# limix/CellRegMap

Hardware: AMD Instinct MI355X
Metric: variant-tests/sec (interaction test) (higher is better)
Workload: dtype f64

## Files before the change

cellregmap_amd/csrc/api_core.hip:

```cpp
#include <dlfcn.h>

#include <algorithm>
#include <atomic>
#include <cstdarg>
#include <mutex>

#include <map>

#include "crm_internal.h"
#include "eigh.h"

namespace crm {

static thread_local std::string g_error;

void set_error(const char* fmt, ...) {
    char buf[1024];
    va_list ap;
    va_start(ap, fmt);
    vsnprintf(buf, sizeof buf, fmt, ap);
    va_end(ap);
    g_error = buf;
}

const char* last_error_text() { return g_error.c_str(); }

namespace {
struct Roctx {
    int (*push)(const char*) = nullptr;
    int (*pop)() = nullptr;
    Roctx() {
        void* h = dlopen("librocprofiler-sdk-roctx.so", RTLD_LAZY | RTLD_GLOBAL);
        if (!h) h = dlopen("librocprofiler-sdk-roctx.so.1", RTLD_LAZY | RTLD_GLOBAL);
        if (!h) return;
        push = reinterpret_cast<int (*)(const char*)>(dlsym(h, "roctxRangePushA"));
        pop = reinterpret_cast<int (*)()>(dlsym(h, "roctxRangePop"));
        if (!push || !pop) push = nullptr, pop = nullptr;
    }
};
const Roctx& roctx() {
    static Roctx r;
    return r;
}
bool ranges_on() {
    static const bool on = getenv("CRM_ROCTX") || getenv("ROCP_TOOL_LIBRARIES") || getenv("ROCPROFILER_LIBRARY_CTOR");
    return on;
}
}

void trace_push(const char* name) {
    if (ranges_on() && roctx().push) roctx().push(name);
}
void trace_pop() {
    if (ranges_on() && roctx().pop) roctx().pop();
}

static bool poison_mode() {
    static const bool on = getenv("CRM_POISON") && atoi(getenv("CRM_POISON")) != 0;
    return on;
}
static constexpr size_t REDZONE = 4096;
static std::atomic<long> g_overruns{0};
long overruns_detected() { return g_overruns.load(); }
static std::atomic<long> g_live_bytes{0};
long live_device_bytes() { return g_live_bytes.load(); }

static void check_redzone(const void* ptr, size_t bytes) {
    if (!ptr || !poison_mode()) return;
    std::vector<unsigned char> rz(REDZONE);
    if (hipMemcpy(rz.data(), static_cast<const char*>(ptr) + bytes, REDZONE, hipMemcpyDeviceToHost) != hipSuccess) return;
    for (size_t i = 0; i < REDZONE; i++) {
        if (rz[i] != 0xFF) {
            g_overruns++;
            fprintf(stderr, "[crm] CRM_POISON: write past the end of a %zu-byte device buffer (first touched byte at +%zu)\n",
                    bytes, i);
            break;
        }
    }
}

static hipStream_t fill_stream() {
    static std::mutex mu;
    static std::map<int, hipStream_t> streams;
    int dev = 0;
    if (hipGetDevice(&dev) != hipSuccess) return nullptr;
    std::lock_guard<std::mutex> lock(mu);
    auto it = streams.find(dev);
    if (it != streams.end()) return it->second;
    hipStream_t st = nullptr;
    if (hipStreamCreateWithFlags(&st, hipStreamNonBlocking) != hipSuccess) st = nullptr;
    streams[dev] = st;
    return st;
}

int DevBuf::ensure(size_t need) {
    if (need <= bytes) return CRM_OK;
    if (ptr) {
        check_redzone(ptr, bytes);
        CRM_HIP(hipFree(ptr));
        g_live_bytes -= (long)bytes;
        ptr = nullptr;
        bytes = 0;
    }
    const size_t total = need + REDZONE;
    hipError_t e = hipMalloc(&ptr, total);
    if (e == hipErrorOutOfMemory && trim_idle_workspaces() > 0) {
        (void)hipGetLastError();
        e = hipMalloc(&ptr, total);
    }
    if (e != hipSuccess) {
        ptr = nullptr;
        (void)hipGetLastError();
        set_error("device allocation of %zu bytes failed: %s", need, hipGetErrorString(e));
        return CRM_ERR_HIP;
    }
    bytes = need;
    static std::atomic<unsigned long> allocations{0};
    serial = ++allocations;
    g_live_bytes += (long)need;
    hipStream_t fs = fill_stream();
    CRM_HIP(hipMemsetAsync(ptr, poison_mode() ? 0xFF : 0, total, fs));
    CRM_HIP(hipStreamSynchronize(fs));
    return CRM_OK;
}

static std::mutex g_ctx_mutex;
static std::vector<crm_ctx*> g_contexts;

static size_t trim_context(crm_ctx* c) {
    if (!c->eigh_ws || c->eigh_ws_busy) return 0;
    size_t freed = 0;
    for (const DevBuf* b : {&c->eigh_ws->A, &c->eigh_ws->Vt, &c->eigh_ws->Vc, &c->eigh_ws->QA, &c->eigh_ws->QB}) freed += b->bytes;
    *c->eigh_ws = EighWork();
    return freed;
}

EighWork* acquire_eigh_workspace(crm_ctx* c) {
    std::lock_guard<std::mutex> lock(g_ctx_mutex);
    if (!c->eigh_ws) c->eigh_ws = new EighWork();
    c->eigh_ws_busy = true;
    return c->eigh_ws;
}

void release_eigh_workspace(crm_ctx* c) {
    std::lock_guard<std::mutex> lock(g_ctx_mutex);
    c->eigh_ws_busy = false;
}

size_t trim_idle_workspaces() {
    std::lock_guard<std::mutex> lock(g_ctx_mutex);
    size_t freed = 0;
    for (crm_ctx* c : g_contexts) freed += trim_context(c);
    return freed;
}
void DevBuf::release() {
    if (ptr) check_redzone(ptr, bytes);
    if (ptr) (void)hipFree(ptr);
    g_live_bytes -= (long)bytes;
    ptr = nullptr;
    bytes = 0;
    serial = 0;
}

int upload_padded(hipStream_t st, double* dst, long ld_dst, long rows_pad, const double* src,
                  long ld_src, long rows, long cols) {
    CRM_HIP(hipMemsetAsync(dst, 0, sizeof(double) * rows_pad * ld_dst, st));
    if (rows > 0 && cols > 0)
        CRM_HIP(hipMemcpy2DAsync(dst, ld_dst * sizeof(double), src, ld_src * sizeof(double),
                                 cols * sizeof(double), rows, hipMemcpyHostToDevice, st));
    return CRM_OK;
}

}

using namespace crm;

extern "C" {

const char* crm_last_error(void) { return last_error_text(); }
const char* crm_version(void) { return "0.6.0"; }

int crm_ctx_create(int device, crm_ctx** out) {
    return crm::guarded("crm_ctx_create", [&]() -> int {
    if (!out) return CRM_ERR_ARG;
    *out = nullptr;
    int count = 0;
    CRM_HIP(hipGetDeviceCount(&count));
    if (device < 0 || device >= count) {
        set_error("crm_ctx_create: device %d not present (%d visible)", device, count);
        return CRM_ERR_ARG;
    }
    CRM_HIP(hipSetDevice(device));
    crm_ctx* c = new crm_ctx();
    c->device = device;
    if (const char* e = getenv("CRM_KIN_ROUTE")) c->kin_route = std::max(0, std::min(2, atoi(e)));
    CRM_HIP(hipStreamCreateWithFlags(&c->stream, hipStreamNonBlocking));
    CRM_HIP(hipStreamCreateWithFlags(&c->upload_stream, hipStreamNonBlocking));
    CRM_HIP(hipEventCreate(&c->ev0));
    CRM_HIP(hipEventCreate(&c->ev1));
    int prio_least = 0, prio_greatest = 0;
    CRM_HIP(hipDeviceGetStreamPriorityRange(&prio_least, &prio_greatest));
    CRM_HIP(hipStreamCreateWithPriority(&c->side_stream, hipStreamNonBlocking, prio_least));
    for (hipEvent_t* e : {&c->ev_fork, &c->ev_side, &c->ev_main, &c->ev_fits}) CRM_HIP(hipEventCreateWithFlags(e, hipEventDisableTiming));
    {
        std::lock_guard<std::mutex> lock(g_ctx_mutex);
        g_contexts.push_back(c);
    }
    *out = c;
    return CRM_OK;
    });
}

int crm_ctx_trim(crm_ctx* c) {
    return crm::guarded_on("crm_ctx_trim", c, [&]() -> int {
    if (!c) return CRM_ERR_ARG;
    CRM_HIP(hipSetDevice(c->device));
    CRM_HIP(hipStreamSynchronize(c->stream));
    if (c->side_stream) CRM_HIP(hipStreamSynchronize(c->side_stream));
    std::lock_guard<std::mutex> lock(g_ctx_mutex);
    (void)trim_context(c);
    return CRM_OK;
    });
}

void crm_ctx_destroy(crm_ctx* c) {
    try {
    if (!c) return;
    (void)hipSetDevice(c->device);
    (void)hipStreamSynchronize(c->stream);
    if (c->side_stream) (void)hipStreamSynchronize(c->side_stream);
    {
        std::lock_guard<std::mutex> lock(g_ctx_mutex);
        g_contexts.erase(std::remove(g_contexts.begin(), g_contexts.end(), c), g_contexts.end());
        delete c->eigh_ws;
        c->eigh_ws = nullptr;
    }
    c->replay_clear();
    for (auto* b : c->all_bufs()) b->release();
    for (auto& e : c->timed) {
        (void)hipEventDestroy(e.first);
        (void)hipEventDestroy(e.second);
    }
    (void)hipEventDestroy(c->ev0);
    (void)hipEventDestroy(c->ev1);
    for (hipEvent_t e : {c->ev_fork, c->ev_side, c->ev_main, c->ev_fits})
        if (e) (void)hipEventDestroy(e);
    if (c->side_stream) (void)hipStreamDestroy(c->side_stream);
    (void)hipStreamDestroy(c->stream);
    if (c->upload_stream) (void)hipStreamDestroy(c->upload_stream);
    if (c->sync_timeouts_host) (void)hipHostFree(c->sync_timeouts_host);
    delete c;
    } catch (...) {
    }
}

int crm_ctx_synchronize(crm_ctx* c) {
    return crm::guarded_on("crm_ctx_synchronize", c, [&]() -> int {
    if (!c) return CRM_ERR_ARG;
    CRM_HIP(hipSetDevice(c->device));
    CRM_HIP(hipStreamSynchronize(c->stream));
    if (c->side_stream) CRM_HIP(hipStreamSynchronize(c->side_stream));
    return CRM_OK;
    });
}

int crm_set_block_variants(crm_ctx* c, int variants) {
    return crm::guarded_on("crm_set_block_variants", c, [&]() -> int {
    if (!c || variants < 0) return CRM_ERR_ARG;
    c->block_variants = variants == 0 ? 0 : (int)round_up(variants, 128);
    return CRM_OK;
    });
}

int crm_set_null_fit_polish(crm_ctx* c, int on) {
    return crm::guarded_on("crm_set_null_fit_polish", c, [&]() -> int {
    if (!c) return CRM_ERR_ARG;
    c->polish = on != 0;
    return CRM_OK;
    });
}

int crm_set_progress_callback(crm_ctx* c, void (*callback)(long, long, void*), void* user) {
    return crm::guarded_on("crm_set_progress_callback", c, [&]() -> int {
    if (!c) return CRM_ERR_ARG;
    if (callback) c->progress[std::this_thread::get_id()] = crm_ctx::Progress{callback, user};
    else c->progress.erase(std::this_thread::get_id());
    return CRM_OK;
    });
}

int crm_set_fast_rotation(crm_ctx* c, int on) {
    return crm::guarded_on("crm_set_fast_rotation", c, [&]() -> int {
    if (!c) return CRM_ERR_ARG;
    c->fast_T = on != 0;
    return CRM_OK;
    });
}

extern "C++" {
namespace crm {
namespace {
struct FormSlot { const char* name; int value; bool set; };
FormSlot g_forms[] = {{"gram_staged", 0, false}, {"kr_no_tail", 0, false}, {"nullfit_per_wave", 0, false}, {"kin_fold", 0, false},
                      {"eigh_one_stage", 0, false}, {"nullfit_exact", 0, false}, {"donor_pairs", 0, false},
                      {"pairs_without_kinship_term", 0, false}, {"flat_kappa_milli", 0, false}, {"chase_abort", 0, false}, {"nullfit_one_per_wave", 0, false},
                      {"kin_diag", 0, false}, {"donor_pairs_rotate", 0, false}, {"rho0_positions", 0, false},
                      {"rotation_tails", 0, false}, {"woodbury_ytY", 0, false},
                      {"wb_block_order", 0, false}, {"block_fused", 0, false}, {"wb_gram_fused", 0, false},
                      {"gram_strips", 0, false}, {"side_stream", 0, false}};
std::mutex g_forms_mu;
}
int form(const char* name, int otherwise) {
    std::lock_guard<std::mutex> lock(g_forms_mu);
    for (const FormSlot& f : g_forms)
        if (strcmp(f.name, name) == 0) return f.set ? f.value : otherwise;
    return otherwise;
}
}
}

int crm_test_set_form(const char* name, int value, int reset) {
    return crm::guarded("crm_test_set_form", [&]() -> int {
    if (!name) return CRM_ERR_ARG;
    std::lock_guard<std::mutex> lock(crm::g_forms_mu);
    for (crm::FormSlot& f : crm::g_forms)
        if (strcmp(f.name, name) == 0) {
            f.value = value;
            f.set = reset == 0;
            return CRM_OK;
        }
    crm::set_error("crm_test_set_form: no kernel form is called '%s'", name);
    return CRM_ERR_ARG;
    });
}

long crm_test_tail_launches(const crm_ctx* ctx) { return ctx ? ctx->tail_launches : -1; }

long crm_test_spectrum_tail_launches(const crm_ctx* ctx) { return ctx ? ctx->spectrum_tail_launches : -1; }

long crm_test_dense_repeats(const crm_ctx* ctx) { return ctx ? ctx->dense_repeats : -1; }

long crm_test_donor_pair_blocks(const crm_ctx* ctx) { return ctx ? ctx->donor_pair_blocks : -1; }

int crm_test_gram_dma_launches(const crm_ctx* ctx, long* launches) {
    return crm::guarded("crm_test_gram_dma_launches", [&]() -> int {
    if (!ctx || !launches) return CRM_ERR_ARG;
    *launches = ctx->gram_dma_launches;
    return CRM_OK;
    });
}
int crm_test_unrelated_donor_blocks(const crm_ctx* ctx, long* blocks) {
    return crm::guarded("crm_test_unrelated_donor_blocks", [&]() -> int {
    if (!ctx || !blocks) return CRM_ERR_ARG;
    *blocks = ctx->unrelated_donor_blocks;
    return CRM_OK;
    });
}

int crm_test_fused_blocks(const crm_ctx* ctx, long* blocks) {
    return crm::guarded("crm_test_fused_blocks", [&]() -> int {
    if (!ctx || !blocks) return CRM_ERR_ARG;
    *blocks = ctx->fused_blocks;
    return CRM_OK;
    });
}

int crm_test_wb_gram_fused_blocks(const crm_ctx* ctx, long* blocks) {
    return crm::guarded("crm_test_wb_gram_fused_blocks", [&]() -> int {
    if (!ctx || !blocks) return CRM_ERR_ARG;
    *blocks = ctx->wb_gram_fused_blocks;
    return CRM_OK;
    });
}

int crm_test_side_stream_blocks(const crm_ctx* ctx, long* blocks) {
    return crm::guarded("crm_test_side_stream_blocks", [&]() -> int {
    if (!ctx || !blocks) return CRM_ERR_ARG;
    *blocks = ctx->side_stream_blocks;
    return CRM_OK;
    });
}

int crm_test_rho0_position_blocks(const crm_ctx* ctx, long* blocks) {
    return crm::guarded("crm_test_rho0_position_blocks", [&]() -> int {
    if (!ctx || !blocks) return CRM_ERR_ARG;
    *blocks = ctx->rho0_position_blocks;
    return CRM_OK;
    });
}
int crm_test_rotation_tail_launches(const crm_ctx* ctx, long* launches) {
    return crm::guarded("crm_test_rotation_tail_launches", [&]() -> int {
    if (!ctx || !launches) return CRM_ERR_ARG;
    *launches = ctx->rotation_tail_launches;
    return CRM_OK;
    });
}

long crm_test_tests_without_pair(const crm_ctx* ctx) { return ctx ? ctx->tests_without_pair : -1; }

int crm_test_set_shared_h(crm_ctx* ctx, int mode) {
    return crm::guarded_on("crm_test_set_shared_h", ctx, [&]() -> int {
    if (!ctx) return CRM_ERR_ARG;
    ctx->tune.shared_h = mode < 0 ? -1 : (mode > 0 ? 1 : 0);
    return CRM_OK;
    });
}

int crm_kernel_timer_reset(crm_ctx* c) {
    return crm::guarded_on("crm_kernel_timer_reset", c, [&]() -> int {
    if (!c) return CRM_ERR_ARG;
    CRM_HIP(hipSetDevice(c->device));
    CRM_HIP(hipStreamSynchronize(c->stream));
    c->timed_used = 0;
    c->kr_flops = 0.0;
    c->timing = true;
    return CRM_OK;
    });
}

int crm_kernel_timer_stop(crm_ctx* c) {
    return crm::guarded_on("crm_kernel_timer_stop", c, [&]() -> int {
    if (!c) return CRM_ERR_ARG;
    c->timing = false;
    return CRM_OK;
    });
}

int crm_kernel_timer_read(crm_ctx* c, double* kr_ms, long* kr_launches, double* kr_flops,
                          double* total_ms) {
    return crm::guarded_on("crm_kernel_timer_read", c, [&]() -> int {
    if (!c) return CRM_ERR_ARG;
    CRM_HIP(hipSetDevice(c->device));
    CRM_HIP(hipStreamSynchronize(c->stream));
    double ms = 0.0;
    for (size_t i = 0; i < c->timed_used; i++) {
        float t = 0.f;
        CRM_HIP(hipEventElapsedTime(&t, c->timed[i].first, c->timed[i].second));
        ms += t;
    }
    if (kr_ms) *kr_ms = ms;
    if (kr_launches) *kr_launches = (long)c->timed_used;
    if (kr_flops) *kr_flops = c->kr_flops;
    if (total_ms) *total_ms = 0.0;
    return CRM_OK;
    });
}

int crm_test_set_contraction(crm_ctx* c, int tile_width, int lds_dma) {
    return crm::guarded_on("crm_test_set_contraction", c, [&]() -> int {
    if (!c || (tile_width != 0 && tile_width != 64 && tile_width != 128 && tile_width != 160)) return CRM_ERR_ARG;
    c->tune.bn = tile_width;
    c->tune.glds = lds_dma ? 1 : 0;
    return CRM_OK;
    });
}

long crm_test_sync_fallbacks(const crm_ctx* c) { return c ? c->sync_fallbacks : -1; }
long crm_test_overruns(void) { return crm::overruns_detected(); }
long crm_test_live_device_bytes(void) { return crm::live_device_bytes(); }

int crm_test_set_kinship_route(crm_ctx* c, int on) {
    return crm::guarded_on("crm_test_set_kinship_route", c, [&]() -> int {
    if (!c) return CRM_ERR_ARG;
    c->kin_route = on < 0 ? 0 : (on > 2 ? 2 : on);
    return CRM_OK;
    });
}

int crm_test_overrun_selftest(crm_ctx* c) {
    return crm::guarded_on("crm_test_overrun_selftest", c, [&]() -> int {
    if (!c) return CRM_ERR_ARG;
    CRM_HIP(hipSetDevice(c->device));
    const long before = overruns_detected();
    {
        DevBuf b;
        CRM_TRY(b.ensure(1000));
        if (poison_mode()) CRM_HIP(hipMemset(static_cast<char*>(b.ptr) + 1000, 0, 8));
        CRM_HIP(hipDeviceSynchronize());
    }
    return (int)(overruns_detected() - before);
    });
}

int crm_test_check_context(crm_ctx* c) {
    return crm::guarded_on("crm_test_check_context", c, [&]() -> int {
    if (!c) return CRM_ERR_ARG;
    CRM_HIP(hipSetDevice(c->device));
    CRM_HIP(hipStreamSynchronize(c->stream));
    for (const DevBuf* b : c->all_bufs()) check_redzone(b->ptr, b->bytes);
    if (c->eigh_ws)
        for (const DevBuf* b : {&c->eigh_ws->A, &c->eigh_ws->Vt, &c->eigh_ws->Vc, &c->eigh_ws->QA, &c->eigh_ws->QB, &c->eigh_ws->d,
                                &c->eigh_ws->e, &c->eigh_ws->tau, &c->eigh_ws->lam, &c->eigh_ws->small})
            check_redzone(b->ptr, b->bytes);
    return CRM_OK;
    });
}

int crm_test_null_fit_probe(crm_ctx* c, int on, double x) {
    return crm::guarded_on("crm_test_null_fit_probe", c, [&]() -> int {
    if (!c) return CRM_ERR_ARG;
    if (on < 0 || on > 2) return CRM_ERR_ARG;
    c->probe_on = on != 0;
    c->probe_mode = on;
    c->probe_x = x;
    return CRM_OK;
    });
}

int crm_test_null_fit_probe_read(crm_ctx* c, double* out, long capacity) {
    return crm::guarded_on("crm_test_null_fit_probe_read", c, [&]() -> int {
    if (!c || !out || capacity < (long)c->probe_out.size()) return CRM_ERR_ARG;
    std::copy(c->probe_out.begin(), c->probe_out.end(), out);
    return (int)c->probe_out.size();
    });
}

int crm_test_set_contraction_sync(crm_ctx* c, int every) {
    return crm::guarded_on("crm_test_set_contraction_sync", c, [&]() -> int {
    if (!c || every < 0) return CRM_ERR_ARG;
    c->tune.sync = every;
    return CRM_OK;
    });
}

int crm_test_contract(crm_ctx* c, long cells, int M, int N, const double* X, const double* Y,
                      double* C, int ksplit) {
    return crm::guarded_on("crm_test_contract", c, [&]() -> int {
    if (!c || cells <= 0 || M <= 0 || N <= 0 || !X || !Y || !C || ksplit < 1) return CRM_ERR_ARG;
    CRM_HIP(hipSetDevice(c->device));
    const long cp = round_up(cells, GEMM_BK * (long)ksplit);
    const long ldx = round_up(M, 128), ldy = round_up(N, 128);
    DevBuf bx, by, bc, bp;
    CRM_TRY(bx.ensure(sizeof(double) * cp * ldx));
    CRM_TRY(by.ensure(sizeof(double) * cp * ldy));
    const long cstride = (long)M * ldy;
    CRM_TRY(bc.ensure(sizeof(double) * cstride * ksplit));
    CRM_TRY(bp.ensure(sizeof(GemmProblem)));
    CRM_TRY(upload_padded(c->stream, bx.as<double>(), ldx, cp, X, M, cells, M));
    CRM_TRY(upload_padded(c->stream, by.as<double>(), ldy, cp, Y, N, cells, N));
    GemmProblem p{};
    p.X = bx.as<double>(); p.Y = by.as<double>(); p.C = bc.as<double>();
    p.ldx = ldx; p.ldy = ldy; p.ldc = ldy; p.M = M; p.N = N;
    CRM_HIP(hipMemcpyAsync(bp.ptr, &p, sizeof p, hipMemcpyHostToDevice, c->stream));
    CRM_TRY(launch_gemm_tn(c, bp.as<GemmProblem>(), 1, M, N, cp, false, 0, ksplit, cstride));
    CRM_TRY(launch_reduce_splits(c->stream, bc.as<double>(), cstride, ksplit, cstride));
    CRM_HIP(hipMemcpy2DAsync(C, N * sizeof(double), bc.ptr, ldy * sizeof(double), N * sizeof(double),
                             M, hipMemcpyDeviceToHost, c->stream));
    CRM_HIP(hipStreamSynchronize(c->stream));
    return CRM_OK;
    });
}

int crm_test_contract_kr(crm_ctx* c, long cells, int B, int k0, int N, const double* G,
                         const double* E, const double* Y, double* C) {
    return crm::guarded_on("crm_test_contract_kr", c, [&]() -> int {
    if (!c || cells <= 0 || B <= 0 || k0 <= 0 || N <= 0 || !G || !E || !Y || !C) return CRM_ERR_ARG;
    CRM_HIP(hipSetDevice(c->device));
    const long cp = round_up(cells, GEMM_BK);
    const long ldg = round_up(B, 128) + 128, lde = round_up(k0, 32), ldy = round_up(N, 128);
    const int M = B * k0;
    DevBuf bg, be, by, bc, bp;
    CRM_TRY(bg.ensure(sizeof(double) * cp * ldg));
    CRM_TRY(be.ensure(sizeof(double) * cp * lde));
    CRM_TRY(by.ensure(sizeof(double) * cp * ldy));
    CRM_TRY(bc.ensure(sizeof(double) * (long)M * ldy));
    CRM_TRY(bp.ensure(sizeof(GemmProblem)));
    CRM_TRY(upload_padded(c->stream, bg.as<double>(), ldg, cp, G, B, cells, B));
    CRM_TRY(upload_padded(c->stream, be.as<double>(), lde, cp, E, k0, cells, k0));
    CRM_TRY(upload_padded(c->stream, by.as<double>(), ldy, cp, Y, N, cells, N));
    GemmProblem p{};
    p.X = bg.as<double>(); p.E = be.as<double>(); p.Y = by.as<double>(); p.C = bc.as<double>();
    p.ldx = ldg; p.lde = lde; p.ldy = ldy; p.ldc = ldy; p.M = M; p.N = N; p.k0 = k0;
    CRM_HIP(hipMemcpyAsync(bp.ptr, &p, sizeof p, hipMemcpyHostToDevice, c->stream));
    CRM_TRY(launch_gemm_tn(c, bp.as<GemmProblem>(), 1, M, N, cp, true, k0, 1, 0));
    CRM_HIP(hipMemcpy2DAsync(C, N * sizeof(double), bc.ptr, ldy * sizeof(double), N * sizeof(double),
                             M, hipMemcpyDeviceToHost, c->stream));
    CRM_HIP(hipStreamSynchronize(c->stream));
    return CRM_OK;
    });
}

int crm_test_contract_kr_t(crm_ctx* c, long cells, int B, int k0, int N, const double* G, const double* E,
                           const double* Y, double* CT) {
    return crm::guarded_on("crm_test_contract_kr_t", c, [&]() -> int {
    if (!c || cells <= 0 || B <= 0 || k0 <= 0 || N <= 0 || !G || !E || !Y || !CT) return CRM_ERR_ARG;
    CRM_HIP(hipSetDevice(c->device));
    const long cp = round_up(cells, GEMM_BK);
    const long ldg = round_up(B, 128) + 128, lde = round_up(k0, 32), ldy = round_up(N, 128);
    const int M = B * k0;
    const long ldc = round_up(M, 128);
    DevBuf bg, be, by, bc, bp;
    CRM_TRY(bg.ensure(sizeof(double) * cp * ldg));
    CRM_TRY(be.ensure(sizeof(double) * cp * lde));
    CRM_TRY(by.ensure(sizeof(double) * cp * ldy));
    CRM_TRY(bc.ensure(sizeof(double) * (long)N * ldc));
    CRM_TRY(bp.ensure(sizeof(GemmProblem)));
    CRM_TRY(upload_padded(c->stream, bg.as<double>(), ldg, cp, G, B, cells, B));
    CRM_TRY(upload_padded(c->stream, be.as<double>(), lde, cp, E, k0, cells, k0));
    CRM_TRY(upload_padded(c->stream, by.as<double>(), ldy, cp, Y, N, cells, N));
    GemmProblem p{};
    p.X = bg.as<double>(); p.E = be.as<double>(); p.Y = by.as<double>(); p.C = bc.as<double>();
    p.ldx = ldg; p.lde = lde; p.ldy = ldy; p.ldc = ldc; p.M = M; p.N = N; p.k0 = k0;
    CRM_HIP(hipMemcpyAsync(bp.ptr, &p, sizeof p, hipMemcpyHostToDevice, c->stream));
    CRM_TRY(launch_kr_transposed(c, bp.as<GemmProblem>(), 1, M, N, cp, k0));
    CRM_HIP(hipMemcpy2DAsync(CT, M * sizeof(double), bc.ptr, ldc * sizeof(double), M * sizeof(double), N,
                             hipMemcpyDeviceToHost, c->stream));
    CRM_HIP(hipStreamSynchronize(c->stream));
    return CRM_OK;
    });
}

}

#include "nullfit.h"

extern "C" {

int crm_test_eigvalsh(crm_ctx* c, int count, int k, const double* F, double* lambda) {
    return crm::guarded_on("crm_test_eigvalsh", c, [&]() -> int {
    if (!c || count <= 0 || k <= 0 || !F || !lambda) return CRM_ERR_ARG;
    CRM_HIP(hipSetDevice(c->device));
    DevBuf bF, bQ, bL, bP;
    CRM_TRY(bF.ensure(sizeof(double) * (size_t)count * k * k));
    CRM_TRY(bQ.ensure(sizeof(double) * count));
    CRM_TRY(bL.ensure(sizeof(double) * (size_t)count * k));
    CRM_TRY(bP.ensure(sizeof(double) * count));
    CRM_HIP(hipMemcpyAsync(bF.ptr, F, sizeof(double) * (size_t)count * k * k, hipMemcpyHostToDevice, c->stream));
    CRM_HIP(hipMemsetAsync(bQ.ptr, 0, sizeof(double) * count, c->stream));
    DevBuf bS;
    CRM_TRY(bS.ensure(sizeof(double) * eig_scratch_doubles(count, k)));
    CRM_TRY(launch_eig_davies(c->stream, bF.as<double>(), bQ.as<double>(), count, k, bL.as<double>(),
                              bP.as<double>(), nullptr, nullptr, true, bS.as<double>()));
    CRM_HIP(hipMemcpyAsync(lambda, bL.ptr, sizeof(double) * (size_t)count * k, hipMemcpyDeviceToHost, c->stream));
    CRM_HIP(hipStreamSynchronize(c->stream));
    return CRM_OK;
    });
}

static int davies_hook(crm_ctx* c, int count, int k, const double* Q, const double* lambda, double* pvalue, int* ifault,
                       double* liu, int* trace) {
    if (!c || count <= 0 || k <= 0 || !Q || !lambda || !pvalue) return CRM_ERR_ARG;
    CRM_HIP(hipSetDevice(c->device));
    DevBuf bQ, bL, bP, bI, bU, bT;
    if (trace) CRM_TRY(bT.ensure(sizeof(int) * 3 * (size_t)count));
    CRM_TRY(bQ.ensure(sizeof(double) * count));
    CRM_TRY(bL.ensure(sizeof(double) * (size_t)count * k));
    CRM_TRY(bP.ensure(sizeof(double) * count));
    CRM_TRY(bI.ensure(sizeof(int) * count));
    CRM_TRY(bU.ensure(sizeof(double) * count));
    CRM_HIP(hipMemcpyAsync(bQ.ptr, Q, sizeof(double) * count, hipMemcpyHostToDevice, c->stream));
    CRM_HIP(hipMemcpyAsync(bL.ptr, lambda, sizeof(double) * (size_t)count * k, hipMemcpyHostToDevice, c->stream));
    CRM_TRY(launch_eig_davies(c->stream, nullptr, bQ.as<double>(), count, k, bL.as<double>(), bP.as<double>(),
                              bI.as<int>(), bU.as<double>(), false, nullptr, trace ? bT.as<int>() : nullptr));
    CRM_HIP(hipMemcpyAsync(pvalue, bP.ptr, sizeof(double) * count, hipMemcpyDeviceToHost, c->stream));
    if (ifault) CRM_HIP(hipMemcpyAsync(ifault, bI.ptr, sizeof(int) * count, hipMemcpyDeviceToHost, c->stream));
    if (liu) CRM_HIP(hipMemcpyAsync(liu, bU.ptr, sizeof(double) * count, hipMemcpyDeviceToHost, c->stream));
    if (trace) CRM_HIP(hipMemcpyAsync(trace, bT.ptr, sizeof(int) * 3 * (size_t)count, hipMemcpyDeviceToHost, c->stream));
    CRM_HIP(hipStreamSynchronize(c->stream));
    return CRM_OK;
}

int crm_test_davies(crm_ctx* c, int count, int k, const double* Q, const double* lambda, double* pvalue,
                    int* ifault, double* liu) {
    return crm::guarded_on("crm_test_davies", c, [&]() -> int {
    return davies_hook(c, count, k, Q, lambda, pvalue, ifault, liu, nullptr);
    });
}

int crm_test_davies_trace(crm_ctx* c, int count, int k, const double* Q, const double* lambda, double* pvalue,
                          int* ifault, double* liu, int* trace) {
    return crm::guarded_on("crm_test_davies_trace", c, [&]() -> int {
    if (!trace) return CRM_ERR_ARG;
    return davies_hook(c, count, k, Q, lambda, pvalue, ifault, liu, trace);
    });
}

int crm_test_tail_pvalue(crm_ctx* c, int count, int k, const double* Q, const double* lambda, double* pvalue,
                         double* logp, int* status) {
    return crm::guarded_on("crm_test_tail_pvalue", c, [&]() -> int {
    if (!c || count <= 0 || k <= 0 || !Q || !lambda || !pvalue || !logp || !status) return CRM_ERR_ARG;
    CRM_HIP(hipSetDevice(c->device));
    DevBuf bQ, bL, bP, bG, bS;
    CRM_TRY(bQ.ensure(sizeof(double) * count));
    CRM_TRY(bL.ensure(sizeof(double) * (size_t)count * k));
    CRM_TRY(bP.ensure(sizeof(double) * count));
    CRM_TRY(bG.ensure(sizeof(double) * count));
    CRM_TRY(bS.ensure(sizeof(int) * count));
    CRM_HIP(hipMemcpyAsync(bQ.ptr, Q, sizeof(double) * count, hipMemcpyHostToDevice, c->stream));
    CRM_HIP(hipMemcpyAsync(bL.ptr, lambda, sizeof(double) * (size_t)count * k, hipMemcpyHostToDevice, c->stream));
    CRM_TRY(launch_tail_pvalue(c->stream, bQ.as<double>(), bL.as<double>(), count, k, bP.as<double>(), bG.as<double>(),
                               bS.as<int>()));
    CRM_HIP(hipMemcpyAsync(pvalue, bP.ptr, sizeof(double) * count, hipMemcpyDeviceToHost, c->stream));
    CRM_HIP(hipMemcpyAsync(logp, bG.ptr, sizeof(double) * count, hipMemcpyDeviceToHost, c->stream));
    CRM_HIP(hipMemcpyAsync(status, bS.ptr, sizeof(int) * count, hipMemcpyDeviceToHost, c->stream));
    CRM_HIP(hipStreamSynchronize(c->stream));
    return CRM_OK;
    });
}

int crm_test_lrt_logp(crm_ctx* c, int count, const double* lrs, double* logp) {
    return crm::guarded_on("crm_test_lrt_logp", c, [&]() -> int {
    if (!c || count <= 0 || !lrs || !logp) return CRM_ERR_ARG;
    CRM_HIP(hipSetDevice(c->device));
    DevBuf bX, bG;
    CRM_TRY(bX.ensure(sizeof(double) * count));
    CRM_TRY(bG.ensure(sizeof(double) * count));
    CRM_HIP(hipMemcpyAsync(bX.ptr, lrs, sizeof(double) * count, hipMemcpyHostToDevice, c->stream));
    CRM_TRY(launch_lrt_logp(c->stream, bX.as<double>(), count, bG.as<double>()));
    CRM_HIP(hipMemcpyAsync(logp, bG.ptr, sizeof(double) * count, hipMemcpyDeviceToHost, c->stream));
    CRM_HIP(hipStreamSynchronize(c->stream));
    return CRM_OK;
    });
}

}
```

cellregmap_amd/csrc/wb_gram_fused.hip:

```cpp
#include <type_traits>

#include "assemble.h"
#include "gram_common.h"

namespace crm {

namespace {

constexpr int WF_MAXQ_P = 10, WF_MAXQ_O = 9, WF_PSUM = 6;
constexpr int WF_UW = 56;

}

WbFusedLayout wb_gram_fused_layout(int k0, int KT, long ldp) {
    WbFusedLayout L;
    const int KS = (k0 + 3) / 4;
    L.urows = 4 * KS;
    L.UW = WF_UW;
    L.RS = (k0 + 4) | 2;
    L.nP = (int)(ldp / 128);
    L.nU = (L.urows * (L.UW / 2) + 63) / 64;
    L.rows_o = KT - k0;
    L.nO = (L.rows_o * (L.RS / 2) + 63) / 64;
    L.off_P = k0 * L.RS + L.nO * 128;
    L.off_U = L.off_P + L.nP * 128;
    L.off_S0 = L.off_U + L.nU * 128;
    L.off_d = L.off_S0 + 128;
    L.off_rp = L.off_d + 64;
    L.total = L.off_rp + ((L.rows_o + 1) & ~1);
    return L;
}

namespace {

template <int NTL, bool STRIPS>
__global__ __launch_bounds__(256, NTL <= 7 ? 2 : 1) void wb_gram_fused_kernel(AssembleArgs a, WbFusedArgs f, WbFusedLayout L, int KT) {
    constexpr int NTILES = NTL * (NTL + 1) / 2, MAXT = (NTILES + 3) / 4;
    constexpr int MAXKS = 14;
    extern __shared__ __align__(16) double smem[];
    double* const img = smem;
    double* const Pl = smem + L.off_P;
    double* const Ul = smem + L.off_U;
    double* const S0l = smem + L.off_S0;
    double* const dS = smem + L.off_d;
    const double** const rowp = reinterpret_cast<const double**>(smem + L.off_rp);
    const int b = blockIdx.x;
    const NullFitOut fit = a.fit[b];
    const AssembleRho R = a.rho[fit.rho_index];
    const double ratio = fit.v0 / fit.v1;
    const bool has_A = a.sorted_pos[b] >= 0;
    const int tid = threadIdx.x;
    const int lane = tid & 63, wave = __builtin_amdgcn_readfirstlane(tid >> 6);
    const int l15 = lane & 15, lq = lane >> 4;
    const int k0 = a.k0, RS = L.RS;
    constexpr int UW = WF_UW;
    const int npair = k0 * (k0 + 1) / 2, KS = (k0 + 3) / 4, JT = (k0 + 15) / 16;
    const int D = f.donors, Ptot = D * k0;
    const double* __restrict__ zeros = a.A_none;

    for (int e = tid; e < k0 * RS; e += 256) img[e] = 0.0;
    for (int t = tid; t < L.rows_o; t += 256) rowp[t] = gram_other_row(a, R, b, t);
    const int nPU = L.nP + L.nU + 1;
    int poff[WF_MAXQ_P], ocode[WF_MAXQ_O];
#pragma unroll
    for (int q = 0; q < WF_MAXQ_P; q++) {
        const int I = wave + 4 * q;
        if (I < L.nP) poff[q] = 128 * I + 2 * lane;
        else if (I < L.nP + L.nU) {
            const int u = 64 * (I - L.nP) + lane, k = u / (UW / 2), cu = u - k * (UW / 2);
            poff[q] = k < L.urows ? k * (int)f.ldu + 2 * cu : 0;
        } else poff[q] = 2 * lane;
    }
#pragma unroll
    for (int q = 0; q < WF_MAXQ_O; q++) {
        const int u = 64 * (wave + 4 * q) + lane, t = u / (RS / 2), cu = u - t * (RS / 2);
        ocode[q] = t < L.rows_o ? (t << 8) | (2 * cu) : -1;
    }
    auto chunk = [&](int d, int& start, int& end, int& c0, int& lim) __attribute__((always_inline)) {
        start = (k0 * d) & ~3;
        end = d + 1 < D ? (k0 * (d + 1)) & ~3 : (Ptot + 3) & ~3;
        c0 = 2 - (k0 * d - start);
        lim = end < Ptot ? end : Ptot;
    };
    auto issue_pus = [&](int d) __attribute__((always_inline)) {
        int start, end, c0, lim;
        chunk(d, start, end, c0, lim);
        const double* __restrict__ Pd = f.P + (size_t)d * f.p_slab + (long)b * f.ldp;
        const double* __restrict__ Ud = f.U + (size_t)d * f.u_slab;
        const double* __restrict__ S0 = R.S0 + (start - c0);
#pragma unroll
        for (int q = 0; q < WF_MAXQ_P; q++) {
            const int I = wave + 4 * q;
            if (I < L.nP) gram_dma16(Pd + poff[q], Pl + 128 * I);
            else if (I < L.nP + L.nU) gram_dma16(Ud + poff[q], Ul + 128 * (I - L.nP));
            else if (I < nPU) {
                const int col = poff[q];
                gram_dma16(col >= c0 && start - c0 + col < lim ? S0 + col : zeros, S0l);
            }
        }
    };
    auto issue_others = [&](int d) __attribute__((always_inline)) {
        int start, end, c0, lim;
        chunk(d, start, end, c0, lim);
        const int shift = start - c0;
#pragma unroll
        for (int q = 0; q < WF_MAXQ_O; q++) {
            const int I = wave + 4 * q;
            if (I < L.nO) {
                const int code = ocode[q], col = code & 255;
                const bool in = code >= 0 && col >= c0 && shift + col < lim;
                const double* src = zeros;
                if (in) src = rowp[code >> 8] + (shift + col);
                gram_dma16(src, img + k0 * RS + 128 * I);
            }
        }
    };
    const int iw = 16 * wave + l15;
    int pidx[16];
#pragma unroll
    for (int ks = 0; ks < 16; ks++) {
        const int k = 4 * ks + lq, lo = k < iw ? k : iw, hi = k < iw ? iw : k;
        pidx[ks] = k < k0 && iw < k0 ? lo * k0 - lo * (lo - 1) / 2 + (hi - lo) : 0;
    }
    const int first = gram_wave_first(wave, b);
    const int ntw = gram_wave_ntiles<NTL, STRIPS>(first);
    int t_i[MAXT], t_j[MAXT], t_ij[MAXT], r_off[NTL];
#pragma unroll
    for (int i = 0; i < NTL; i++) {
        const int row = 16 * i + l15;
        r_off[i] = (row < KT ? row : 0) * RS + lq;
    }
    if constexpr (!STRIPS) {
        gram_wave_tiles<NTL, false>(first, t_ij);
#pragma unroll
        for (int t = 0; t < MAXT; t++) {
            const int ri = 16 * (t_ij[t] & 255) + l15, rj = 16 * (t_ij[t] >> 8) + l15;
            t_i[t] = (ri < KT ? ri : 0) * RS + lq;
            t_j[t] = (rj < KT ? rj : 0) * RS + lq;
        }
    }
    v4d acc[MAXT];
#pragma unroll
    for (int t = 0; t < MAXT; t++) acc[t] = (v4d){0.0, 0.0, 0.0, 0.0};
    double psum[WF_PSUM];
#pragma unroll
    for (int q = 0; q < WF_PSUM; q++) psum[q] = 0.0;
    const int per = (D + f.splits - 1) / f.splits;
    int split = 0;

    auto gram = [&](int col0, int nks, auto nt_tag) __attribute__((always_inline)) {
        constexpr int NT = decltype(nt_tag)::value;
        const double* __restrict__ S = img + col0;
        const double* __restrict__ Dw = dS + col0 + lq;
        double fa[NT], fr[NT];
        double dk = Dw[0];
#pragma unroll
        for (int t = 0; t < NT; t++) {
            fa[t] = S[t_i[t]];
            fr[t] = S[t_j[t]];
        }
        for (int ks = 0; ks < nks; ks++) {
            const bool more = ks + 1 < nks;
            const int nx = more ? 4 * (ks + 1) : 4 * ks;
            const double dn = Dw[nx];
#pragma unroll
            for (int t = 0; t < NT; t++) {
                acc[t] = __builtin_amdgcn_mfma_f64_16x16x4f64(fa[t], fr[t] * dk, acc[t], 0, 0, 0);
                fa[t] = S[t_i[t] + nx];
                fr[t] = S[t_j[t] + nx];
            }
            dk = dn;
        }
    };
    auto gram_strips = [&](int col0, int nks, auto role_tag) __attribute__((always_inline)) {
        constexpr int ROLE = decltype(role_tag)::value;
        constexpr int NT = kStripDeal<NTL>.n[ROLE];
        const double* __restrict__ S = img + col0;
        const double* __restrict__ Dw = dS + col0 + lq;
        const double* rows[NTL];
        double fr[NTL], fw[NTL];
        static_for<0, NTL>([&](auto ic) {
            constexpr int i = decltype(ic)::value;
            if constexpr (kStripDeal<NTL>.reads(ROLE, i)) {
                rows[i] = S + r_off[i];
                fr[i] = rows[i][0];
            }
        });
        double dk = Dw[0];
        auto step = [&](int off) __attribute__((always_inline)) {
            static_for<0, NTL>([&](auto jc) {
                constexpr int j = decltype(jc)::value;
                if constexpr (kStripDeal<NTL>.is_b(ROLE, j)) {
                    fw[j] = fr[j] * dk;
                    if constexpr (kStripDeal<NTL>.last_a(ROLE, j) < 0) fr[j] = rows[j][off + 4];
                }
            });
            static_for<0, NT>([&](auto tc) {
                constexpr int t = decltype(tc)::value;
                acc[t] = __builtin_amdgcn_mfma_f64_16x16x4f64(fr[kStripDeal<NTL>.ti[ROLE][t]], fw[kStripDeal<NTL>.tj[ROLE][t]], acc[t], 0, 0, 0);
                static_for<0, NTL>([&](auto ic) {
                    constexpr int i = decltype(ic)::value;
                    if constexpr (kStripDeal<NTL>.last_a(ROLE, i) == t) fr[i] = rows[i][off + 4];
                });
            });
            dk = Dw[off + 4];
        };
        static_for<0, MAXKS>([&](auto kc) {
            constexpr int ks = decltype(kc)::value;
            if (ks < nks) step(4 * ks);
        });
    };

    __syncthreads();
    issue_pus(0);
    issue_others(0);
    dma_barrier();
    for (int d = 0; d < D; d++) {
        int start, end, c0, lim;
        chunk(d, start, end, c0, lim);
        if (tid < RS) dS[tid] = gram_weight(ratio, S0l[tid]);
#pragma unroll
        for (int q = 0; q < WF_PSUM; q++)
            if (tid + 256 * q < npair) psum[q] += Pl[tid + 256 * q];
        if (d + 1 == D || d + 1 == (split + 1) * per) {
            double* __restrict__ out = f.Psum + (size_t)split * f.psum_slab + (long)b * f.ldp;
#pragma unroll
            for (int q = 0; q < WF_PSUM; q++)
                if (tid + 256 * q < npair) { out[tid + 256 * q] = psum[q]; psum[q] = 0.0; }
            split++;
        }
        if (has_A && wave < JT) {
            unsigned uo = (unsigned)(lq * UW + l15);
            asm volatile("" : "+v"(uo));
            const double* __restrict__ ub = Ul + uo;
            const int jcut = end - k0 * d;
#pragma unroll
            for (int th = 0; th < 4; th += 2) {
                if (th < JT) {
                    v4d cr[2];
#pragma unroll
                    for (int t = 0; t < 2; t++) cr[t] = (v4d){0.0, 0.0, 0.0, 0.0};
                    double af[3], bf[3][2];
                    auto frag = [&](int ks, int slot) __attribute__((always_inline)) {
                        af[slot] = Pl[pidx[ks]];
#pragma unroll
                        for (int t = 0; t < 2; t++)
                            if (th + t < JT) bf[slot][t] = ub[4 * ks * UW + 16 * (th + t)];
                    };
                    frag(0, 0);
                    if (1 < KS) frag(1, 1);
#pragma unroll
                    for (int ks = 0; ks < 16; ks++) {
                        if (ks < KS) {
                            if (ks + 2 < KS) frag(ks + 2, (ks + 2) % 3);
#pragma unroll
                            for (int t = 0; t < 2; t++)
                                if (th + t < JT)
                                    cr[t] = __builtin_amdgcn_mfma_f64_16x16x4f64(af[ks % 3], bf[ks % 3][t], cr[t], 0, 0, 0);
                            __builtin_amdgcn_sched_barrier(0);
                        }
                    }
#pragma unroll
                    for (int reg = 0; reg < 4; reg++) {
                        const int r = 16 * wave + lq + 4 * reg;
                        if (r < k0) {
#pragma unroll
                            for (int t = 0; t < 2; t++) {
                                const int j = 16 * (th + t) + l15;
                                if (th + t < JT && j < k0) img[r * RS + (j < jcut ? j + 2 : j - jcut)] = cr[t][reg];
                            }
                        }
                    }
                }
            }
        }
        dma_barrier();
        if (d + 1 < D) issue_pus(d + 1);
        const int nks = (end - start) / 4;
        if constexpr (STRIPS) {
            if (nks > 0) {
                if (first == 0) gram_strips(c0, nks, std::integral_constant<int, 0>{});
                else if (first == 1) gram_strips(c0, nks, std::integral_constant<int, 1>{});
                else if (first == 2) gram_strips(c0, nks, std::integral_constant<int, 2>{});
                else gram_strips(c0, nks, std::integral_constant<int, 3>{});
            }
        } else {
            if (ntw == MAXT) gram(c0, nks, std::integral_constant<int, MAXT>{});
            else gram(c0, nks, std::integral_constant<int, MAXT - 1>{});
        }
        dma_barrier();
        if (d + 1 < D) issue_others(d + 1);
    }
    for (; split < f.splits; split++) {
        double* __restrict__ out = f.Psum + (size_t)split * f.psum_slab + (long)b * f.ldp;
        for (int e = tid; e < npair; e += 256) out[e] = 0.0;
    }
    if constexpr (STRIPS) gram_wave_tiles<NTL, true>(first, t_ij);
    gram_store_tiles(a.wb_Gw + (long)b * KT * KT, KT, t_ij, ntw, acc, lq, l15);
}

bool aligned16(const void* p) { return (reinterpret_cast<uintptr_t>(p) & 15) == 0; }

}

bool wb_gram_fused_serves(const AssembleArgs& a, const WbFusedArgs& f, int nrho) {
    const int k0 = a.k0, KT = k0 + a.c + 2 + a.wb_k1, ts = (KT + 15) / 16;
    if (form("wb_gram_fused", 1) == 0 || form("gram_staged", 0) != 0) return false;
    if (a.wb_k1 <= 0 || k0 % 2 != 0 || !donor_pairs_rotate_serves(k0) || ts < 5 || ts > 8 || f.donors < 1 || f.splits < 1) return false;
    if (f.ldp % 128 != 0 || f.ldp < k0 * (k0 + 1) / 2 || f.p_slab % 2 != 0 || f.u_slab % 2 != 0 || f.ldu % 2 != 0 || f.ldu < 4 * ((k0 + 3) / 4) ||
        f.k2pad < 4 * ((k0 + 3) / 4) || !aligned16(f.P) || !aligned16(f.U) || !aligned16(a.A_none) || !a.wb_Gw)
        return false;
    if (a.wb_ldR % 2 != 0 || !aligned16(a.wb_R)) return false;
    for (int i = 0; i < nrho; i++) {
        const AssembleRho& R = a.rho[i];
        if (R.r != f.donors * k0 || R.ldW % 2 != 0 || R.ldT % 2 != 0 || !aligned16(R.ty) || !aligned16(R.tW) || !aligned16(R.T) ||
            !aligned16(R.S0))
            return false;
    }
    const WbFusedLayout L = wb_gram_fused_layout(k0, KT, f.ldp);
    return L.nP + L.nU + 1 <= 4 * WF_MAXQ_P && L.nO <= 4 * WF_MAXQ_O && L.RS <= 64 && k0 * (k0 + 1) / 2 <= 256 * WF_PSUM &&
           sizeof(double) * (size_t)L.total <= 160 * 1024;
}

int launch_wb_gram_fused(hipStream_t st, const AssembleArgs& a, const WbFusedArgs& f, int nrho, int variants) {
    if (variants <= 0) return CRM_OK;
    if (!wb_gram_fused_serves(a, f, nrho)) {
        set_error("fused unrelated-donor Gram: k0=%d, c=%d outside the supported range", a.k0, a.c);
        return CRM_ERR_INTERNAL;
    }
    const int KT = a.k0 + a.c + 2 + a.wb_k1, ts = (KT + 15) / 16;
    const WbFusedLayout L = wb_gram_fused_layout(a.k0, KT, f.ldp);
    const size_t lds = sizeof(double) * (size_t)L.total;
    const bool strips = form("gram_strips", 1) != 0;
    auto fused = [&](auto ntl) {
        constexpr int NTL = decltype(ntl)::value;
        return strips ? launch_with_lds(wb_gram_fused_kernel<NTL, true>, dim3(variants), dim3(256), lds, st, true, a, f, L, KT)
                      : launch_with_lds(wb_gram_fused_kernel<NTL, false>, dim3(variants), dim3(256), lds, st, true, a, f, L, KT);
    };
    if (ts == 5) CRM_HIP(fused(std::integral_constant<int, 5>{}));
    else if (ts == 6) CRM_HIP(fused(std::integral_constant<int, 6>{}));
    else if (ts == 7) CRM_HIP(fused(std::integral_constant<int, 7>{}));
    else CRM_HIP(fused(std::integral_constant<int, 8>{}));
    return CRM_OK;
}

}
```

Baseline: 81880.

## Interleave next-chunk DMA pieces among MFMA k-steps in fused Gram kernel

Adds a SPREAD variant of the fused unrelated-donor Gram kernel, enabled by default whenever strips are on. Instead of issuing all P/U/S0 and other-row async copies in bursts between barriers, each copy piece is placed between MFMA steps of the strip Gram and the weighted-image loop, with sched_barrier pins holding the order. The aim is to hide global-to-LDS transfer latency behind matrix math. In exchange it adds register pressure, extra scheduling constraints, and more complex bounds logic.

```diff
diff --git a/cellregmap_amd/csrc/api_core.hip b/cellregmap_amd/csrc/api_core.hip
--- a/cellregmap_amd/csrc/api_core.hip
+++ b/cellregmap_amd/csrc/api_core.hip
@@ -307,7 +307,7 @@
                       {"kin_diag", 0, false}, {"donor_pairs_rotate", 0, false}, {"rho0_positions", 0, false},
                       {"rotation_tails", 0, false}, {"woodbury_ytY", 0, false},
                       {"wb_block_order", 0, false}, {"block_fused", 0, false}, {"wb_gram_fused", 0, false},
-                      {"gram_strips", 0, false}, {"side_stream", 0, false}};
+                      {"gram_strips", 0, false}, {"side_stream", 0, false}, {"wb_gram_spread", 0, false}};
 std::mutex g_forms_mu;
 }
 int form(const char* name, int otherwise) {
diff --git a/cellregmap_amd/csrc/wb_gram_fused.hip b/cellregmap_amd/csrc/wb_gram_fused.hip
--- a/cellregmap_amd/csrc/wb_gram_fused.hip
+++ b/cellregmap_amd/csrc/wb_gram_fused.hip
@@ -8,6 +8,7 @@
 namespace {
 
 constexpr int WF_MAXQ_P = 10, WF_MAXQ_O = 9, WF_PSUM = 6;
+constexpr int WF_PIN = 0x2 | 0x4 | 0x80 | 0x100 | 0x200;
 constexpr int WF_UW = 56;
 
 }
@@ -33,8 +34,9 @@
 
 namespace {
 
-template <int NTL, bool STRIPS>
+template <int NTL, bool STRIPS, bool SPREAD>
 __global__ __launch_bounds__(256, NTL <= 7 ? 2 : 1) void wb_gram_fused_kernel(AssembleArgs a, WbFusedArgs f, WbFusedLayout L, int KT) {
+    static_assert(STRIPS || !SPREAD, "the pieces are spread among the k-steps of the strip deal only");
     constexpr int NTILES = NTL * (NTL + 1) / 2, MAXT = (NTILES + 3) / 4;
     constexpr int MAXKS = 14;
     extern __shared__ __align__(16) double smem[];
@@ -74,7 +76,13 @@
 #pragma unroll
     for (int q = 0; q < WF_MAXQ_O; q++) {
         const int u = 64 * (wave + 4 * q) + lane, t = u / (RS / 2), cu = u - t * (RS / 2);
-        ocode[q] = t < L.rows_o ? (t << 8) | (2 * cu) : -1;
+        ocode[q] = t < L.rows_o ? (t << 8) | (2 * cu) : (SPREAD ? 255 : -1);
+    }
+    const int nPsi = L.nP + L.nU;
+    unsigned pbyte[WF_MAXQ_P];
+    if constexpr (SPREAD) {
+#pragma unroll
+        for (int q = 0; q < WF_MAXQ_P; q++) pbyte[q] = 8u * (unsigned)poff[q];
     }
     auto chunk = [&](int d, int& start, int& end, int& c0, int& lim) __attribute__((always_inline)) {
         start = (k0 * d) & ~3;
@@ -113,6 +121,53 @@
                 if (in) src = rowp[code >> 8] + (shift + col);
                 gram_dma16(src, img + k0 * RS + 128 * I);
             }
+        }
+    };
+    const char* Pnext = nullptr;
+    const char* Unext = nullptr;
+    int n_next = 0;
+    auto set_next = [&](int d) __attribute__((always_inline)) {
+        Pnext = reinterpret_cast<const char*>(f.P + (size_t)d * f.p_slab + (long)b * f.ldp);
+        Unext = reinterpret_cast<const char*>(f.U + (size_t)d * f.u_slab);
+        n_next = d < D ? nPsi : 0;
+    };
+    auto pu_piece = [&](auto qc) __attribute__((always_inline)) {
+        constexpr int q = decltype(qc)::value;
+        if constexpr (q < WF_MAXQ_P) {
+            int I = wave + 4 * q;
+            asm volatile("" : "+s"(I));
+            if (I < n_next) {
+                unsigned off = pbyte[q];
+                asm volatile("" : "+v"(off));
+                gram_dma16(reinterpret_cast<const double*>((I < L.nP ? Pnext : Unext) + off), Pl + 128 * I);
+            }
+        }
+    };
+    auto s0_piece = [&](int d) __attribute__((always_inline)) {
+        if (d < D && ((nPsi - wave) & 3) == 0) {
+            int start, end, c0, lim;
+            chunk(d, start, end, c0, lim);
+            const int col = 2 * lane;
+            gram_dma16(col >= c0 && start - c0 + col < lim ? R.S0 + (start - c0) + col : zeros, S0l);
+        }
+    };
+    int n_other = 0, o_c0 = 0, o_shift = 0, o_width = 0;
+    auto set_others = [&](int d, bool on) __attribute__((always_inline)) {
+        int start, end, lim;
+        chunk(d, start, end, o_c0, lim);
+        o_shift = start - o_c0;
+        o_width = lim - start;
+        n_other = on ? L.nO : 0;
+    };
+    auto other_row = [&](int q) __attribute__((always_inline)) { return rowp[ocode[q] >> 8]; };
+    auto other_piece = [&](int q, const double* row) __attribute__((always_inline)) {
+        int I = wave + 4 * q;
+        asm volatile("" : "+s"(I));
+        if (I < n_other) {
+            const int col = ocode[q] & 255;
+            const double* src = row + (unsigned)(o_shift + col);
+            asm volatile("" : "+v"(src));
+            gram_dma16((unsigned)(col - o_c0) < (unsigned)o_width ? src : zeros, img + k0 * RS + 128 * I);
         }
     };
     const int iw = 16 * wave + l15;
@@ -187,7 +242,7 @@
             }
         });
         double dk = Dw[0];
-        auto step = [&](int off) __attribute__((always_inline)) {
+        auto step = [&](int off, auto kc) __attribute__((always_inline)) {
             static_for<0, NTL>([&](auto jc) {
                 constexpr int j = decltype(jc)::value;
                 if constexpr (kStripDeal<NTL>.is_b(ROLE, j)) {
@@ -198,6 +253,11 @@
             static_for<0, NT>([&](auto tc) {
                 constexpr int t = decltype(tc)::value;
                 acc[t] = __builtin_amdgcn_mfma_f64_16x16x4f64(fr[kStripDeal<NTL>.ti[ROLE][t]], fw[kStripDeal<NTL>.tj[ROLE][t]], acc[t], 0, 0, 0);
+                if constexpr (SPREAD && t == 0) {
+                    __builtin_amdgcn_sched_barrier(WF_PIN);
+                    pu_piece(kc);
+                    __builtin_amdgcn_sched_barrier(WF_PIN);
+                }
                 static_for<0, NTL>([&](auto ic) {
                     constexpr int i = decltype(ic)::value;
                     if constexpr (kStripDeal<NTL>.last_a(ROLE, i) == t) fr[i] = rows[i][off + 4];
@@ -207,17 +267,28 @@
         };
         static_for<0, MAXKS>([&](auto kc) {
             constexpr int ks = decltype(kc)::value;
-            if (ks < nks) step(4 * ks);
+            if (ks < nks) step(4 * ks, kc);
+            else if constexpr (SPREAD) pu_piece(kc);
         });
     };
 
     __syncthreads();
-    issue_pus(0);
-    issue_others(0);
+    if constexpr (!SPREAD) {
+        issue_pus(0);
+        issue_others(0);
+    } else {
+        set_next(0);
+        s0_piece(0);
+        static_for<0, WF_MAXQ_P>(pu_piece);
+        set_others(0, true);
+#pragma unroll
+        for (int q = 0; q < WF_MAXQ_O; q++) other_piece(q, other_row(q));
+    }
     dma_barrier();
     for (int d = 0; d < D; d++) {
         int start, end, c0, lim;
         chunk(d, start, end, c0, lim);
+        if constexpr (SPREAD) set_others(d, d > 0);
         if (tid < RS) dS[tid] = gram_weight(ratio, S0l[tid]);
 #pragma unroll
         for (int q = 0; q < WF_PSUM; q++)
@@ -251,12 +322,19 @@
                     if (1 < KS) frag(1, 1);
 #pragma unroll
                     for (int ks = 0; ks < 16; ks++) {
+                        const bool piece = SPREAD && th == 0 && ks < WF_MAXQ_O;
+                        const double* row = nullptr;
+                        if (piece) row = other_row(ks);
                         if (ks < KS) {
                             if (ks + 2 < KS) frag(ks + 2, (ks + 2) % 3);
 #pragma unroll
                             for (int t = 0; t < 2; t++)
                                 if (th + t < JT)
                                     cr[t] = __builtin_amdgcn_mfma_f64_16x16x4f64(af[ks % 3], bf[ks % 3][t], cr[t], 0, 0, 0);
+                            __builtin_amdgcn_sched_barrier(0);
+                        }
+                        if (piece) {
+                            other_piece(ks, row);
                             __builtin_amdgcn_sched_barrier(0);
                         }
                     }
@@ -273,12 +351,20 @@
                     }
                 }
             }
+        } else if constexpr (SPREAD) {
+#pragma unroll
+            for (int q = 0; q < WF_MAXQ_O; q++) other_piece(q, other_row(q));
         }
         dma_barrier();
-        if (d + 1 < D) issue_pus(d + 1);
+        if constexpr (!SPREAD) {
+            if (d + 1 < D) issue_pus(d + 1);
+        } else {
+            set_next(d + 1);
+            s0_piece(d + 1);
+        }
         const int nks = (end - start) / 4;
         if constexpr (STRIPS) {
-            if (nks > 0) {
+            if (SPREAD || nks > 0) {
                 if (first == 0) gram_strips(c0, nks, std::integral_constant<int, 0>{});
                 else if (first == 1) gram_strips(c0, nks, std::integral_constant<int, 1>{});
                 else if (first == 2) gram_strips(c0, nks, std::integral_constant<int, 2>{});
@@ -289,7 +375,9 @@
             else gram(c0, nks, std::integral_constant<int, MAXT - 1>{});
         }
         dma_barrier();
-        if (d + 1 < D) issue_others(d + 1);
+        if constexpr (!SPREAD) {
+            if (d + 1 < D) issue_others(d + 1);
+        }
     }
     for (; split < f.splits; split++) {
         double* __restrict__ out = f.Psum + (size_t)split * f.psum_slab + (long)b * f.ldp;
@@ -332,10 +420,12 @@
     const WbFusedLayout L = wb_gram_fused_layout(a.k0, KT, f.ldp);
     const size_t lds = sizeof(double) * (size_t)L.total;
     const bool strips = form("gram_strips", 1) != 0;
+    const bool spread = strips && form("wb_gram_spread", 1) != 0;
     auto fused = [&](auto ntl) {
         constexpr int NTL = decltype(ntl)::value;
-        return strips ? launch_with_lds(wb_gram_fused_kernel<NTL, true>, dim3(variants), dim3(256), lds, st, true, a, f, L, KT)
-                      : launch_with_lds(wb_gram_fused_kernel<NTL, false>, dim3(variants), dim3(256), lds, st, true, a, f, L, KT);
+        if (spread) return launch_with_lds(wb_gram_fused_kernel<NTL, true, true>, dim3(variants), dim3(256), lds, st, true, a, f, L, KT);
+        return strips ? launch_with_lds(wb_gram_fused_kernel<NTL, true, false>, dim3(variants), dim3(256), lds, st, true, a, f, L, KT)
+                      : launch_with_lds(wb_gram_fused_kernel<NTL, false, false>, dim3(variants), dim3(256), lds, st, true, a, f, L, KT);
     };
     if (ts == 5) CRM_HIP(fused(std::integral_constant<int, 5>{}));
     else if (ts == 6) CRM_HIP(fused(std::integral_constant<int, 6>{}));
```

Result: faster. 83320, median of 6 (+1.8%).
